# omarkhursheed/whisper-sae

Hardware: AMD Instinct MI355X
Metric: activations/sec through SAE train step (d=384->3072, k=32) (higher is better)
Workload: dtype bf16; 1 GPU; BASELINE.json configs[1]: TopKSAE 384->3072 k=32 train step, synthetic activations resident in the HBM ring buffer; batch_per_gpu=16384, global_batch=16384, ring_rows_per_gpu=4194304, parallelism=dp1

## Files before the change

whisper-sae_amd/csrc/wsae_common.h:

```cpp
#pragma once

#include <hip/hip_runtime.h>
#include <stdint.h>
#include <stdio.h>

#include "wsae.h"

void wsae_set_error(const char* fmt, ...);

#define WSAE_HIP_CHECK(expr)                                                              \
    do {                                                                                  \
        hipError_t e_ = (expr);                                                           \
        if (e_ != hipSuccess) {                                                           \
            wsae_set_error("%s failed: %s (%s:%d)", #expr, hipGetErrorString(e_), __FILE__, \
                           __LINE__);                                                     \
            return WSAE_ERR_HIP;                                                          \
        }                                                                                 \
    } while (0)

#define WSAE_REQUIRE(cond, ...)          \
    do {                                 \
        if (!(cond)) {                   \
            wsae_set_error(__VA_ARGS__); \
            return WSAE_ERR_INVALID;     \
        }                                \
    } while (0)

#define WSAE_LAUNCH_CHECK()                                                                  \
    do {                                                                                     \
        hipError_t e_ = hipGetLastError();                                                   \
        if (e_ != hipSuccess) {                                                              \
            wsae_set_error("kernel launch failed: %s (%s:%d)", hipGetErrorString(e_), __FILE__, \
                           __LINE__);                                                        \
            return WSAE_ERR_HIP;                                                             \
        }                                                                                    \
    } while (0)

typedef __bf16 bf16_t;
typedef __bf16 bf16x8 __attribute__((ext_vector_type(8)));
typedef __bf16 bf16x4 __attribute__((ext_vector_type(4)));
typedef float f32x16 __attribute__((ext_vector_type(16)));
typedef float f32x4 __attribute__((ext_vector_type(4)));
typedef float f32x2 __attribute__((ext_vector_type(2)));
typedef __bf16 bf16x2 __attribute__((ext_vector_type(2)));

static inline int64_t ceil_div64(int64_t a, int64_t b) { return (a + b - 1) / b; }
static inline int ceil_div(int a, int b) { return (a + b - 1) / b; }
static inline int64_t align256(int64_t b) { return (b + 255) & ~(int64_t)255; }
__host__ __device__ __forceinline__ int64_t min64(int64_t a, int64_t b) { return a < b ? a : b; }

#define WSAE_MAX_PARTIALS 1024
#define WSAE_WGRAD_MAX_SPLIT 8

struct wsae_prof {
    unsigned mask;
    int max_samples;
    int count[WSAE_K_COUNT];
    hipEvent_t* ev[WSAE_K_COUNT];
};

struct wsae_ctx {
    wsae_prof prof;
    int D, H, K, maxB, prec, device;
    const float* relu_l1w;
    int loss_cols;
    int cus;
    int comm_reserve;
    int64_t P;
    int64_t off[5];
    bf16_t* We_bf16;
    bf16_t* WdT_bf16;
    float* c_fold;
    void* xb;
    void* xT;
    void* gT;
    float* g;
    bf16_t* gb;
    int g_is_bf16;
    int xT_valid;
    int g32_valid;
    float* pre;
    float* smax;
    int smax_valid;
    uint32_t* tmin;
    int tmin_cur;
    int strip_predict;
    int wgrad_sparse;
    float tg_fixed_s;
    int pred_valid;
    const void* pred_x;
    const int32_t* pred_rows;
    float* part_loss;
    float* part_l0;
    float* part_dbd;
    float* part_sq;
    float* colnorm;
    float* wg_slabs;
    float* dbe_slab;
    float* dbpre_part;
    uint32_t* ent_pos;
    void* ent_hid;
    void* ent_dpre;
    int32_t* ent_off;
    int ent_valid;
    const float* ent_vals;
    int ent_B;
    const float* wire_dec_vals;
    int wire_dec_B;
    int32_t* counters;
    int32_t* dead_list;
    int32_t* row_order;
    int resample_max_rows;
    int relu_fp8;
    void* relu_ws;
    int relu_x_B;
    int relu_g_B;
    float* fired;
    const float* wire_metrics;
    int n_dec_blocks;
    int n_sq_parts;
    float* dbd2;
    int32_t* btk_ws;
    int btk_k;
    int btk_mode;
    wsae_batch_topk_state* btk_state;
    size_t ws_bytes;
};

#define WSAE_PROF_BEGIN(ctx, id, st)                                                          \
    const bool prof_on_##id = ((ctx)->prof.mask >> (id)) & 1u &&                               \
                              (ctx)->prof.count[id] < (ctx)->prof.max_samples;                 \
    if (prof_on_##id) (void)hipEventRecord((ctx)->prof.ev[id][2 * (ctx)->prof.count[id]], st)
#define WSAE_PROF_END(ctx, id, st)                                                            \
    if (prof_on_##id) {                                                                       \
        (void)hipEventRecord((ctx)->prof.ev[id][2 * (ctx)->prof.count[id] + 1], st);           \
        (ctx)->prof.count[id]++;                                                              \
    }

#ifdef __HIPCC__

#define WSAE_WAVE 64

template <int M>
__device__ __forceinline__ uint32_t lane_xor_u32(uint32_t x, int lane) {
    if constexpr (M == 1) return (uint32_t)__builtin_amdgcn_update_dpp(0, (int)x, 0xB1, 0xF, 0xF, false);
    else if constexpr (M == 2) return (uint32_t)__builtin_amdgcn_update_dpp(0, (int)x, 0x4E, 0xF, 0xF, false);
    else if constexpr (M == 4) {
        const uint32_t up = (uint32_t)__builtin_amdgcn_update_dpp(0, (int)x, 0x104, 0xF, 0xF, false);
        const uint32_t dn = (uint32_t)__builtin_amdgcn_update_dpp(0, (int)x, 0x114, 0xF, 0xF, false);
        return (lane & 4) ? dn : up;
    } else if constexpr (M == 8) return (uint32_t)__builtin_amdgcn_update_dpp(0, (int)x, 0x128, 0xF, 0xF, false);
    else if constexpr (M == 16) {
        const auto r = __builtin_amdgcn_permlane16_swap((int)x, (int)x, false, false);
        return (uint32_t)((lane & 16) ? r[0] : r[1]);
    } else {
        static_assert(M == 32, "lane_xor_u32: M must be a power of two <= 32");
        const auto r = __builtin_amdgcn_permlane32_swap((int)x, (int)x, false, false);
        return (uint32_t)((lane & 32) ? r[0] : r[1]);
    }
}

__device__ __forceinline__ float wave_sum(float v) {
    const int lane = threadIdx.x & 63;
    v += __uint_as_float(lane_xor_u32<32>(__float_as_uint(v), lane));
    v += __uint_as_float(lane_xor_u32<16>(__float_as_uint(v), lane));
    v += __uint_as_float(lane_xor_u32<8>(__float_as_uint(v), lane));
    v += __uint_as_float(lane_xor_u32<4>(__float_as_uint(v), lane));
    v += __uint_as_float(lane_xor_u32<2>(__float_as_uint(v), lane));
    v += __uint_as_float(lane_xor_u32<1>(__float_as_uint(v), lane));
    return v;
}
__device__ __forceinline__ float wave_max(float v) {
    const int lane = threadIdx.x & 63;
    v = fmaxf(v, __uint_as_float(lane_xor_u32<32>(__float_as_uint(v), lane)));
    v = fmaxf(v, __uint_as_float(lane_xor_u32<16>(__float_as_uint(v), lane)));
    v = fmaxf(v, __uint_as_float(lane_xor_u32<8>(__float_as_uint(v), lane)));
    v = fmaxf(v, __uint_as_float(lane_xor_u32<4>(__float_as_uint(v), lane)));
    v = fmaxf(v, __uint_as_float(lane_xor_u32<2>(__float_as_uint(v), lane)));
    v = fmaxf(v, __uint_as_float(lane_xor_u32<1>(__float_as_uint(v), lane)));
    return v;
}
__device__ __forceinline__ int wave_sum_i(int v) {
    const int lane = threadIdx.x & 63;
    v += (int)lane_xor_u32<32>((uint32_t)v, lane);
    v += (int)lane_xor_u32<16>((uint32_t)v, lane);
    v += (int)lane_xor_u32<8>((uint32_t)v, lane);
    v += (int)lane_xor_u32<4>((uint32_t)v, lane);
    v += (int)lane_xor_u32<2>((uint32_t)v, lane);
    v += (int)lane_xor_u32<1>((uint32_t)v, lane);
    return v;
}
__device__ __forceinline__ int wave_min_i(int v) {
    const int lane = threadIdx.x & 63;
    int o;
    o = (int)lane_xor_u32<32>((uint32_t)v, lane); v = o < v ? o : v;
    o = (int)lane_xor_u32<16>((uint32_t)v, lane); v = o < v ? o : v;
    o = (int)lane_xor_u32<8>((uint32_t)v, lane); v = o < v ? o : v;
    o = (int)lane_xor_u32<4>((uint32_t)v, lane); v = o < v ? o : v;
    o = (int)lane_xor_u32<2>((uint32_t)v, lane); v = o < v ? o : v;
    o = (int)lane_xor_u32<1>((uint32_t)v, lane); v = o < v ? o : v;
    return v;
}

__device__ __forceinline__ float lane_f32(float x, int lane) {
    return __int_as_float(__builtin_amdgcn_readlane(__float_as_int(x), lane));
}
__device__ __forceinline__ double lane_f64(double x, int lane) {
    const long long b = __double_as_longlong(x);
    const unsigned lo = (unsigned)__builtin_amdgcn_readlane((int)(unsigned)b, lane);
    const unsigned hi = (unsigned)__builtin_amdgcn_readlane((int)(unsigned)(b >> 32), lane);
    return __longlong_as_double((long long)(((unsigned long long)hi << 32) | lo));
}

__device__ __forceinline__ float block_sum(float v, float* scratch) {
    v = wave_sum(v);
    const int lane = threadIdx.x & 63, w = threadIdx.x >> 6, nw = blockDim.x >> 6;
    __syncthreads();
    if (lane == 0) scratch[w] = v;
    __syncthreads();
    float r = 0.f;
    if (threadIdx.x == 0)
        for (int i = 0; i < nw; ++i) r += scratch[i];
    return r;
}

#define TICKET_GROUPS 32
#define TICKET_WORDS (1 + TICKET_GROUPS)
__device__ __forceinline__ bool grid_ticket(unsigned long long* t, unsigned payload, unsigned* total) {
    const unsigned nblk = gridDim.x * gridDim.y;
    const unsigned bid = blockIdx.y * gridDim.x + blockIdx.x;
    const unsigned ngrp = nblk < TICKET_GROUPS ? nblk : TICKET_GROUPS;
    const unsigned grp = bid % ngrp;
    const unsigned gsz = (nblk - grp + ngrp - 1) / ngrp;
    const unsigned long long add = (1ull << 32) | payload;
    const unsigned long long o1 = __hip_atomic_fetch_add(t + 1 + grp, add, __ATOMIC_RELAXED, __HIP_MEMORY_SCOPE_AGENT);
    if ((unsigned)(o1 >> 32) != gsz - 1) return false;
    __hip_atomic_store(t + 1 + grp, 0ull, __ATOMIC_RELAXED, __HIP_MEMORY_SCOPE_AGENT);
    const unsigned long long add2 = (1ull << 32) | (unsigned)((o1 + add) & 0xFFFFFFFFull);
    const unsigned long long o2 = __hip_atomic_fetch_add(t, add2, __ATOMIC_RELAXED, __HIP_MEMORY_SCOPE_AGENT);
    if ((unsigned)(o2 >> 32) != ngrp - 1) return false;
// ... 83 lines not shown
```

whisper-sae_amd/csrc/wsae_ctx.hip:

```cpp
#include <stdarg.h>
#include <stdlib.h>
#include <string.h>

#include <new>

#include "wsae_common.h"
#include "wsae_topk.h"
#include <cstdlib>
#include <vector>

static thread_local char g_err[512] = "";
static void prof_free(wsae_ctx* c);

void wsae_set_error(const char* fmt, ...) {
    va_list ap;
    va_start(ap, fmt);
    vsnprintf(g_err, sizeof(g_err), fmt, ap);
    va_end(ap);
}

extern "C" const char* wsae_last_error(void) { return g_err; }
extern "C" int wsae_version(void) { return WSAE_VERSION; }

extern "C" int64_t wsae_param_count(int32_t D, int32_t H) {
    return 2 * (int64_t)D * H + H + 2 * (int64_t)D;
}

extern "C" int wsae_param_offsets(int32_t D, int32_t H, int64_t off[5]) {
    WSAE_REQUIRE(off != nullptr && D > 0 && H > 0, "wsae_param_offsets: bad arguments");
    off[0] = 0;
    off[1] = (int64_t)D * H;
    off[2] = 2 * (int64_t)D * H;
    off[3] = off[2] + H;
    off[4] = off[3] + D;
    return WSAE_OK;
}

namespace {
struct DeviceGuard {
    int prev = -1;
    bool good = false;
    explicit DeviceGuard(int device) {
        if (hipGetDevice(&prev) != hipSuccess) prev = -1;
        good = hipSetDevice(device) == hipSuccess;
    }
    ~DeviceGuard() {
        if (prev >= 0) (void)hipSetDevice(prev);
    }
    bool ok() const { return good; }
};

struct Carver {
    size_t total = 0;
    size_t take(size_t bytes) {
        size_t at = total;
        total += (bytes + 255) & ~(size_t)255;
        return at;
    }
};
}

extern "C" int wsae_ctx_create(const wsae_config* cfg, wsae_ctx** out) {
    WSAE_REQUIRE(cfg && out, "wsae_ctx_create: null argument");
    const int D = cfg->input_dim, H = cfg->hidden_dim, K = cfg->k, maxB = cfg->max_batch;
    WSAE_REQUIRE(D >= 32 && D % 32 == 0 && D <= 2048, "input_dim must be a multiple of 32 in [32,2048], got %d", D);
    WSAE_REQUIRE(H >= 32 && H % 32 == 0, "hidden_dim must be a positive multiple of 32, got %d", H);
    WSAE_REQUIRE(K >= 1 && K <= 128 && K <= H, "k must be in [1, min(128, hidden_dim)], got %d", K);
    WSAE_REQUIRE(maxB >= 1, "max_batch must be >= 1, got %d", maxB);
    WSAE_REQUIRE(cfg->precision == WSAE_PREC_BF16 || cfg->precision == WSAE_PREC_FP32, "unknown precision %d",
                 cfg->precision);
    DeviceGuard guard(cfg->device);
    if (!guard.ok()) {
        wsae_set_error("hipSetDevice(%d) failed", cfg->device);
        return WSAE_ERR_HIP;
    }

    wsae_ctx* c = new (std::nothrow) wsae_ctx();
    if (!c) {
        wsae_set_error("out of host memory");
        return WSAE_ERR_NOMEM;
    }
    memset(c, 0, sizeof(*c));
    c->loss_cols = D;
    c->D = D; c->H = H; c->K = K; c->maxB = maxB; c->prec = cfg->precision; c->device = cfg->device;
    if (hipDeviceGetAttribute(&c->cus, hipDeviceAttributeMultiprocessorCount, cfg->device) != hipSuccess || c->cus < 1)
        c->cus = 256;
    c->P = wsae_param_count(D, H);
    wsae_param_offsets(D, H, c->off);
    c->resample_max_rows = wsae_internal_resample_max_rows(cfg->device);

    const size_t esz = (c->prec == WSAE_PREC_BF16) ? 2 : 4;
    const size_t maxBp = ((size_t)maxB + 127) / 128 * 128;
    Carver cv;
    const size_t o_we = cv.take((size_t)H * D * 2);
    const size_t o_wd = cv.take((size_t)H * D * 2);
    const size_t o_cf = cv.take((size_t)H * 4);
    const size_t o_xb = cv.take((size_t)maxB * D * esz);
    const size_t o_xT = cv.take(maxBp * D * esz);
    const size_t o_gT = cv.take(maxBp * D * esz);
    const size_t o_g = cv.take((size_t)maxB * D * 4);
    const size_t o_gb = cv.take((size_t)maxB * D * 2);
    const size_t o_pre = cv.take((size_t)maxB * H * 4);
    const size_t o_sm = cv.take((size_t)maxB * ((H + 15) / 16) * 4);
    const size_t o_pl = cv.take(WSAE_MAX_PARTIALS * 4);
    const size_t o_p0 = cv.take(WSAE_MAX_PARTIALS * 4);
    const size_t o_pd = cv.take((size_t)WSAE_MAX_PARTIALS * D * 4);
    const size_t o_ps = cv.take((WSAE_MAX_PARTIALS + 64) * 4);
    const size_t o_d2 = cv.take((size_t)64 * D * 4);
    const size_t o_cn = cv.take((size_t)H * 4);
    const size_t o_ct = cv.take((16 + 3 * 2 * TICKET_WORDS) * 4);
    const size_t o_ws = cv.take((size_t)WSAE_WGRAD_MAX_SPLIT * 2 * H * D * 4);
    const size_t o_ds = cv.take((size_t)2 * WSAE_WGRAD_MAX_SPLIT * H * 4);
    const size_t o_dp = cv.take((size_t)((H + 31) / 32) * D * 4);
    const size_t o_ep = cv.take((size_t)maxB * K * 4);
    const size_t o_eh = cv.take((size_t)maxB * K * 4);
    const size_t o_ed = cv.take((size_t)maxB * K * 4);
    const size_t o_eo = cv.take((size_t)((maxB + 31) / 32) * ((H + 127) / 128 + 1) * 4);
    const size_t o_dl = cv.take((size_t)H * 4);
    const size_t o_ro = cv.take((size_t)maxB * 4);
    const size_t o_tm = cv.take(TG_WORDS * 4);
    const size_t o_bt = cv.take(wsae_internal_batch_topk_ws_bytes());
    char* base = nullptr;
    hipError_t e = hipMalloc((void**)&base, cv.total);
    if (e != hipSuccess) {
        wsae_set_error("hipMalloc(%zu bytes of workspace) failed: %s", cv.total, hipGetErrorString(e));
        delete c;
        return WSAE_ERR_NOMEM;
    }
    e = hipMemset(base, 0, cv.total);
    if (e != hipSuccess) {
        wsae_set_error("hipMemset failed: %s", hipGetErrorString(e));
        (void)hipFree(base);
        delete c;
        return WSAE_ERR_HIP;
    }
    c->We_bf16 = (bf16_t*)(base + o_we);
    c->WdT_bf16 = (bf16_t*)(base + o_wd);
    c->c_fold = (float*)(base + o_cf);
    c->xb = base + o_xb;
    c->xT = base + o_xT;
    c->gT = base + o_gT;
    c->g = (float*)(base + o_g);
    c->gb = (bf16_t*)(base + o_gb);
    c->pre = (float*)(base + o_pre);
    c->smax = (float*)(base + o_sm);
    c->part_loss = (float*)(base + o_pl);
    c->part_l0 = (float*)(base + o_p0);
    c->part_dbd = (float*)(base + o_pd);
    c->part_sq = (float*)(base + o_ps);
    c->dbd2 = (float*)(base + o_d2);
    c->colnorm = (float*)(base + o_cn);
    c->counters = (int32_t*)(base + o_ct);
    c->wg_slabs = (float*)(base + o_ws);
    c->dbe_slab = (float*)(base + o_ds);
    c->dbpre_part = (float*)(base + o_dp);
    c->ent_pos = (uint32_t*)(base + o_ep);
    c->ent_hid = base + o_eh;
    c->ent_dpre = base + o_ed;
    c->ent_off = (int32_t*)(base + o_eo);
    c->dead_list = (int32_t*)(base + o_dl);
    c->row_order = (int32_t*)(base + o_ro);
    c->tmin = (uint32_t*)(base + o_tm);
    c->btk_ws = (int32_t*)(base + o_bt);
    const char* sp = getenv("WSAE_STRIP_PREDICT");
    c->strip_predict = (sp && sp[0] == '0') ? 0 : 1;
    const char* ws = getenv("WSAE_WGRAD_SPARSE");
    c->wgrad_sparse = (ws && ws[0] == '0') ? 0 : 1;
    const char* ss = getenv("WSAE_STRIP_SAFETY");
    c->tg_fixed_s = ss ? (float)atof(ss) : 0.f;
    c->ws_bytes = cv.total;
    *out = c;
    return WSAE_OK;
}

extern "C" int wsae_ctx_destroy(wsae_ctx* ctx) {
    if (!ctx) return WSAE_OK;
    prof_free(ctx);
    if (ctx->relu_ws) (void)hipFree(ctx->relu_ws);
    if (ctx->We_bf16) (void)hipFree((void*)ctx->We_bf16);
    delete ctx;
    return WSAE_OK;
}

static const char* const k_names[WSAE_K_COUNT] = {"stage_batch", "encode_gemm", "topk", "decode", "bucket", "wgrad",
                                                  "wgrad_reduce", "sqnorm", "adamw", "rownorm", "prepare", "dead_scan"};

extern "C" const char* wsae_kernel_name(int32_t id) { return (id >= 0 && id < WSAE_K_COUNT) ? k_names[id] : "?"; }

static void prof_free(wsae_ctx* c) {
    for (int k = 0; k < WSAE_K_COUNT; ++k) {
        if (c->prof.ev[k]) {
            for (int i = 0; i < 2 * c->prof.max_samples; ++i) (void)hipEventDestroy(c->prof.ev[k][i]);
            delete[] c->prof.ev[k];
            c->prof.ev[k] = nullptr;
        }
        c->prof.count[k] = 0;
    }
    c->prof.mask = 0;
    c->prof.max_samples = 0;
}

extern "C" int wsae_profile_disable(wsae_ctx* ctx) {
    WSAE_REQUIRE(ctx, "wsae_profile_disable: null ctx");
    prof_free(ctx);
    return WSAE_OK;
}

extern "C" int wsae_profile_enable(wsae_ctx* ctx, int32_t kernel_id, int32_t max_samples) {
    WSAE_REQUIRE(ctx && kernel_id >= -1 && kernel_id < WSAE_K_COUNT && max_samples >= 1 && max_samples <= 65536,
                 "wsae_profile_enable: bad argument");
    prof_free(ctx);
    ctx->prof.max_samples = max_samples;
    for (int k = 0; k < WSAE_K_COUNT; ++k) {
        if (kernel_id != -1 && kernel_id != k) continue;
        ctx->prof.ev[k] = new (std::nothrow) hipEvent_t[2 * (size_t)max_samples];
        if (!ctx->prof.ev[k]) {
            wsae_set_error("out of host memory");
            return WSAE_ERR_NOMEM;
        }
        for (int i = 0; i < 2 * max_samples; ++i) WSAE_HIP_CHECK(hipEventCreate(&ctx->prof.ev[k][i]));
        ctx->prof.mask |= 1u << k;
    }
    return WSAE_OK;
}

extern "C" int wsae_profile_read(wsae_ctx* ctx, int32_t kernel_id, int32_t* n_launches, double* total_ms) {
    WSAE_REQUIRE(ctx && kernel_id >= 0 && kernel_id < WSAE_K_COUNT && n_launches && total_ms,
                 "wsae_profile_read: bad argument");
    *n_launches = 0;
    *total_ms = 0.0;
    if (!ctx->prof.ev[kernel_id]) return WSAE_OK;
    const int n = ctx->prof.count[kernel_id];
    double tot = 0.0;
    for (int i = 0; i < n; ++i) {
        WSAE_HIP_CHECK(hipEventSynchronize(ctx->prof.ev[kernel_id][2 * i + 1]));
        float ms = 0.f;
        WSAE_HIP_CHECK(hipEventElapsedTime(&ms, ctx->prof.ev[kernel_id][2 * i], ctx->prof.ev[kernel_id][2 * i + 1]));
        tot += ms;
    }
    *n_launches = n;
    *total_ms = tot;
    return WSAE_OK;
}

extern "C" int wsae_ctx_set_fired(wsae_ctx* ctx, float* fired) {
    WSAE_REQUIRE(ctx, "wsae_ctx_set_fired: null ctx");
    ctx->fired = fired;
    return WSAE_OK;
}

static uint32_t host_f32_ord(float f) {
    uint32_t u;
    memcpy(&u, &f, 4);
    return (u & 0x80000000u) ? ~u : (u | 0x80000000u);
}
extern "C" int wsae_ctx_set_strip_predict(wsae_ctx* ctx, int32_t on, float assume_store_threshold) {
    WSAE_REQUIRE(ctx, "wsae_ctx_set_strip_predict: null ctx");
    ctx->strip_predict = on ? 1 : 0;
    ctx->pred_valid = 0;
    WSAE_HIP_CHECK(hipDeviceSynchronize());
    const bool forget = assume_store_threshold != assume_store_threshold;
    const float one = 1.0f;
    uint32_t hdr[3] = {forget ? 0u : host_f32_ord(assume_store_threshold), 0u, 0u};
    if (!forget) memcpy(&hdr[1], &one, 4);
    uint32_t* prev = ctx->tmin + ctx->tmin_cur * TG_GROUP_WORDS;
    WSAE_HIP_CHECK(hipMemset(prev, 0, TG_GROUP_WORDS * 4));
    WSAE_HIP_CHECK(hipMemset(ctx->tmin + ((ctx->tmin_cur + 2) % 3) * TG_GROUP_WORDS, 0, TG_GROUP_WORDS * 4));
    WSAE_HIP_CHECK(hipMemcpy(prev, hdr, sizeof(hdr), hipMemcpyHostToDevice));
    return WSAE_OK;
}
extern "C" int wsae_ctx_strip_stats(wsae_ctx* ctx, int64_t* refilled_rows, float* last_min_threshold, float* margin) {
    WSAE_REQUIRE(ctx && refilled_rows && last_min_threshold && margin, "wsae_ctx_strip_stats: null argument");
    std::vector<uint32_t> h(TG_WORDS);
    WSAE_HIP_CHECK(hipDeviceSynchronize());
    WSAE_HIP_CHECK(hipMemcpy(h.data(), ctx->tmin, h.size() * 4, hipMemcpyDeviceToHost));
    *refilled_rows = (int64_t)h[TG_REFILLED];
    uint32_t o = 0xFFFFFFFFu;
    for (int i = 0; i < TG_SLOTS; ++i) {
        const uint32_t s = h[ctx->tmin_cur * TG_GROUP_WORDS + i * TG_SLOT_STRIDE];
        if (s != 0u && s < o) o = s;
    }
    float f = NAN;
    if (o != 0u && o != 0xFFFFFFFFu) {
        const uint32_t u = (o & 0x80000000u) ? (o & 0x7FFFFFFFu) : ~o;
        memcpy(&f, &u, 4);
    }
    *last_min_threshold = f;
    memcpy(margin, &h[ctx->tmin_cur * TG_GROUP_WORDS + TG_HDR_S], 4);
    return WSAE_OK;
}

extern "C" int wsae_ctx_set_wire_metrics(wsae_ctx* ctx, const float* loss_l0) {
    WSAE_REQUIRE(ctx, "wsae_ctx_set_wire_metrics: null ctx");
    ctx->wire_metrics = loss_l0;
    return WSAE_OK;
}

extern "C" int wsae_ctx_set_loss_cols(wsae_ctx* ctx, int32_t cols) {
    WSAE_REQUIRE(ctx && cols >= 1 && cols <= ctx->D, "wsae_ctx_set_loss_cols: columns must be in [1, input_dim]");
    ctx->loss_cols = cols;
    return WSAE_OK;
}

extern "C" size_t wsae_ctx_workspace_bytes(const wsae_ctx* ctx) { return ctx ? ctx->ws_bytes : 0; }

__global__ void __launch_bounds__(256) prepare_kernel(const float* __restrict__ We, const float* __restrict__ WdT,
                                                      const float* __restrict__ be, const float* __restrict__ bpre,
                                                      bf16_t* __restrict__ We16, bf16_t* __restrict__ WdT16,
                                                      float* __restrict__ cfold, int H, int D) {
    const int lane = threadIdx.x & 63;
    const int h = blockIdx.x * 4 + (threadIdx.x >> 6);
    if (h >= H) return;
    const float* row = We + (int64_t)h * D;
    bf16_t* orow = We16 + (int64_t)h * D;
    const float* drow = WdT + (int64_t)h * D;
    bf16_t* odrow = WdT16 + (int64_t)h * D;
    float dot = 0.f;
    for (int d = lane * 4; d < D; d += 256) {
        const float4 wd = *(const float4*)(drow + d);
        bf16x4 o, e;
// ... 31 lines not shown
```

whisper-sae_amd/csrc/wsae_decode_mfma.hip:

```cpp
#include "wsae_chunk_sort.h"
#include "wsae_common.h"
#include "wsae_decode_epilogue.h"
#include "wsae_mfma.h"

#ifdef WSAE_DM_STAMPS
__device__ unsigned long long dm_stamp_sum[8];
#define DM_T(i)                                                                                     \
    {                                                                                               \
        __builtin_amdgcn_sched_barrier(0);                                                          \
        unsigned long long t_;                                                                      \
        asm volatile("s_memtime %0\n\ts_waitcnt lgkmcnt(0)" : "=s"(t_)::"memory");                  \
        __builtin_amdgcn_sched_barrier(0);                                                          \
        dm_acc[i] += t_ - dm_last;                                                                  \
        dm_last = t_;                                                                               \
    }
extern "C" int wsae_debug_stamps(double* out, int reset) {
    unsigned long long h[8];
    if (hipMemcpyFromSymbol(h, HIP_SYMBOL(dm_stamp_sum), sizeof(h)) != hipSuccess) return -1;
    for (int i = 0; i < 8; ++i) out[i] = (double)h[i];
    if (reset) {
        unsigned long long z[8] = {0, 0, 0, 0, 0, 0, 0, 0};
        (void)hipMemcpyToSymbol(HIP_SYMBOL(dm_stamp_sum), z, sizeof(z));
    }
    return 0;
}
#else
#define DM_T(i) __builtin_amdgcn_sched_barrier(0);
#endif

typedef __attribute__((address_space(3))) bf16x4 lds_bf16x4;

__device__ __forceinline__ int dm_sw(int j) { return (j & 15) ^ ((j & 1) ? 12 : 0); }

__device__ __forceinline__ bf16x8 tr_frag(const char* a0, const char* a1) {
    const bf16x4 lo = __builtin_amdgcn_ds_read_tr16_b64_v4bf16((lds_bf16x4*)a0);
    const bf16x4 hi = __builtin_amdgcn_ds_read_tr16_b64_v4bf16((lds_bf16x4*)a1);
    return __builtin_shufflevector(lo, hi, 0, 1, 2, 3, 4, 5, 6, 7);
}

template <int N>
__device__ __forceinline__ void dma_piece(const void* base, const uint32_t (&off)[N], uint32_t lds) {
    static_assert(N == 8 || N == 16, "a piece is 32 or 64 rows");
    const uint32_t l0 = __builtin_amdgcn_readfirstlane(lds);
    uint32_t keep;
#define DP1(i) "global_load_lds_dwordx4 %" #i ", %[b]\n\ts_add_u32 m0, m0, 0x400\n\ts_nop 0\n\t"
    if constexpr (N == 8) {
        asm volatile("s_mov_b32 %[k], m0\n\ts_mov_b32 m0, %[l]\n\ts_nop 0\n\t" DP1(2) DP1(3) DP1(4) DP1(5) DP1(6) DP1(7) DP1(8) DP1(9)
                     "s_mov_b32 m0, %[k]"
                     : [k] "=&s"(keep)
                     : [l] "s"(l0), "v"(off[0]), "v"(off[1]), "v"(off[2]), "v"(off[3]), "v"(off[4]), "v"(off[5]), "v"(off[6]),
                       "v"(off[7]), [b] "s"(base)
                     : "memory");
    } else {
        asm volatile("s_mov_b32 %[k], m0\n\ts_mov_b32 m0, %[l]\n\ts_nop 0\n\t" DP1(2) DP1(3) DP1(4) DP1(5) DP1(6) DP1(7) DP1(8) DP1(9)
                     DP1(10) DP1(11) DP1(12) DP1(13) DP1(14) DP1(15) DP1(16) DP1(17) "s_mov_b32 m0, %[k]"
                     : [k] "=&s"(keep)
                     : [l] "s"(l0), "v"(off[0]), "v"(off[1]), "v"(off[2]), "v"(off[3]), "v"(off[4]), "v"(off[5]), "v"(off[6]),
                       "v"(off[7]), "v"(off[8]), "v"(off[9]), "v"(off[10]), "v"(off[11]), "v"(off[12]), "v"(off[13]),
                       "v"(off[14]), "v"(off[15]), [b] "s"(base)
                     : "memory");
    }
#undef DP1
}

template <int N>
__device__ __forceinline__ void vm_wait() {
    if constexpr (N == 0) asm volatile("s_waitcnt vmcnt(0)" ::: "memory");
    else if constexpr (N == 8) asm volatile("s_waitcnt vmcnt(8)" ::: "memory");
    else {
        static_assert(N == 16, "vm_wait: one piece of 32 or 64 rows in flight");
        asm volatile("s_waitcnt vmcnt(16)" ::: "memory");
    }
}

__host__ __device__ constexpr int dm_wave_bytes(int KS, int D) {
    return 2 * (32 * KS) * 256 + 2 * 2 * (32 * KS) * 4 + D * 2 + 128 * 4;
}

template <int KS, int NSUB, int XDT, bool BWD, int NW>
__global__ void __launch_bounds__(64 * NW, (KS == 1 && NSUB <= 3) ? 2 : 1)
decode_mfma_kernel(const bf16_t* __restrict__ WdT, const float* __restrict__ bd, const float* __restrict__ bpre,
                   const void* __restrict__ x, const int32_t* __restrict__ rows, const float* __restrict__ vals,
                   const int32_t* __restrict__ idx, int B, int K, float* __restrict__ recon_out, float* __restrict__ dpre,
                   float* __restrict__ g32_out, bf16_t* __restrict__ gb_out, int64_t* __restrict__ last_activated,
                   float* __restrict__ fired, const int64_t* __restrict__ step_count, float* __restrict__ part_loss,
                   float* __restrict__ part_l0, float* __restrict__ part_dbd, int32_t* __restrict__ ticket,
                   wsae_stats* __restrict__ stats, int loss_cols, int ntiles, int tw, uint32_t* __restrict__ ent_pos,
                   bf16_t* __restrict__ ent_hid, bf16_t* __restrict__ ent_dpre, int32_t* __restrict__ ent_off) {
    static_assert(NW == 4 || (NW == 8 && BWD), "the chunked form exists for the training backward only");
    constexpr int D = 128 * NSUB;
    constexpr int KP = 32 * KS;
    constexpr int E = KP / 4;
    constexpr int SLOT = KP * 256;
    constexpr int WAVE_BYTES = dm_wave_bytes(KS, D);
    static_assert(WAVE_BYTES % 16 == 0, "per-wave LDS regions stay 16-byte aligned");
    extern __shared__ __attribute__((aligned(16))) char smem[];
    const int lane = threadIdx.x & 63, wave = threadIdx.x >> 6;
    const int n = lane & 15, grp = lane >> 4;
    const uint32_t piece_mask[3] = {n == 0 ? 0xFFFFFFFFu : 0u, n == 1 ? 0xFFFFFFFFu : 0u, n == 2 ? 0xFFFFFFFFu : 0u};
    char* wbase = smem + wave * WAVE_BYTES;
    char* slot0 = wbase;
    char* code = wbase + 2 * SLOT;
    bf16_t* grow = (bf16_t*)(code + 2 * 2 * KP * 4);
    float* stage = (float*)(grow + D);
    float* red = (float*)(smem + NW * WAVE_BYTES);
    int* flag_s = (int*)(red + 8);
    float* dbd_s = (float*)smem;
    const uint32_t slot_lds = (uint32_t)(uintptr_t)(__attribute__((address_space(3))) char*)slot0;

    for (int i = lane; i < 2 * 2 * KP; i += 64) ((int*)code)[i] = 0;
    f32x2 bsum2[NSUB];
#pragma unroll
    for (int s = 0; s < NSUB; ++s) {
        const float2 a = *(const float2*)(bd + 128 * s + 2 * lane), p = *(const float2*)(bpre + 128 * s + 2 * lane);
        bsum2[s] = f32x2{a.x + p.x, a.y + p.y};
    }

    const float scale = 2.0f / ((float)B * (float)loss_cols);
    const int64_t step = (last_activated && step_count) ? *step_count : 0;
    constexpr bool x_bf16 = XDT == WSAE_DT_BF16;
    int tr_off[KS][2], tr_swz[2], a2_off[2 * KS], a2_swz[2 * KS];
    {
        const int i = n >> 2, p = n & 3;
#pragma unroll
        for (int h2 = 0; h2 < 2; ++h2) {
            const int jr = 8 * grp + i + 4 * h2;
            tr_swz[h2] = (dm_sw(jr) ^ (p >> 1)) << 4;
#pragma unroll
            for (int q = 0; q < KS; ++q) tr_off[q][h2] = (32 * q + jr) * 256 + 8 * (p & 1);
        }
#pragma unroll
        for (int m = 0; m < 2 * KS; ++m) {
            a2_off[m] = (16 * m + n) * 256;
            a2_swz[m] = (dm_sw(16 * m + n) ^ grp) << 4;
        }
    }
    float loss_acc = 0.f;
    int l0_acc = 0;
    f32x2 dbd[NSUB];
#pragma unroll
    for (int s = 0; s < NSUB; ++s) dbd[s] = f32x2{0.f, 0.f};

    auto get_code = [&](int bb, int cb) {
        float* vs = (float*)(code + cb * 2 * KP * 4);
        int32_t* is = (int32_t*)(vs + KP);
        if (lane < K) {
            vs[lane] = vals[(int64_t)bb * K + lane];
            is[lane] = idx[(int64_t)bb * K + lane];
        }
    };
    auto sources = [&](int cb, uint32_t (&rp)[E]) {
        const int32_t* is = (const int32_t*)(code + cb * 2 * KP * 4) + KP;
#pragma unroll
        for (int e = 0; e < E; ++e) {
            const int j = 4 * e + grp;
            rp[e] = (uint32_t)is[j] * (uint32_t)D + 8u * (uint32_t)(n ^ dm_sw(j));
        }
    };
    auto issue = [&](const uint32_t (&rp)[E], int s, int slot) {
        asm volatile("s_waitcnt lgkmcnt(0)" ::: "memory");
        uint32_t off[E];
#pragma unroll
        for (int e = 0; e < E; ++e) off[e] = 2u * rp[e] + 256u * (uint32_t)s;
        dma_piece<E>(WdT, off, slot_lds + slot * SLOT);
    };

    const int b_first = NW == 8 ? blockIdx.x * 64 + wave : blockIdx.x * 4 + wave;
    const int b_step = NW == 8 ? 8 : gridDim.x * 4;
    const int b_end = NW == 8 ? min(B, (int)blockIdx.x * 64 + 64) : B;
    int buf = 0, par = 0;
    int64_t src_next = 0;
    uint32_t rowp[E];
#ifdef WSAE_DM_STAMPS
    unsigned long long dm_acc[8] = {0, 0, 0, 0, 0, 0, 0, 0}, dm_last = __builtin_amdgcn_s_memtime();
#endif
    if (b_first < b_end) {
        src_next = rows ? (int64_t)rows[b_first] : (int64_t)b_first;
        get_code(b_first, 0);
        sources(0, rowp);
        issue(rowp, 0, 0);
        if (NSUB > 1) issue(rowp, 1, 1);
    }
    DM_T(0)
    for (int b = b_first; b < b_end; b += b_step) {
        const float* vs = (const float*)(code + buf * 2 * KP * 4);
        const int32_t* is = (const int32_t*)(vs + KP);
        const bool more = b + b_step < b_end;
        {
            const float v = lane < KP ? vs[lane < KP ? lane : 0] : 0.f;
            const bool on = lane < K && v > 0.f;
            l0_acc += __popcll(__ballot(on));
            if (on && last_activated) {
                const int f = is[lane];
                last_activated[f] = step;
                if (fired) fired[f] = 1.f;
            }
        }
        const int64_t src = src_next;
        if (more) src_next = rows ? (int64_t)rows[b + b_step] : (int64_t)(b + b_step);
        uint32_t xraw[NSUB][x_bf16 ? 1 : 2];
#pragma unroll
        for (int s = 0; s < NSUB; ++s) {
            if constexpr (x_bf16) {
                xraw[s][0] = *(const uint32_t*)((const uint16_t*)x + src * D + 128 * s + 2 * lane);
            } else {
                const uint2 t2 = *(const uint2*)((const uint32_t*)x + src * D + 128 * s + 2 * lane);
                xraw[s][0] = t2.x;
                xraw[s][1] = t2.y;
            }
        }
        bf16x8 a1[KS];
#pragma unroll
        for (int q = 0; q < KS; ++q) {
            const float4 v0 = *(const float4*)(vs + 32 * q + 8 * grp), v1 = *(const float4*)(vs + 32 * q + 8 * grp + 4);
            const float vv[8] = {v0.x, v0.y, v0.z, v0.w, v1.x, v1.y, v1.z, v1.w};
            uint32_t w4[4];
#pragma unroll
            for (int p2 = 0; p2 < 4; ++p2) {
                const float a = __builtin_amdgcn_fmed3f(vv[2 * p2], 0.f, INFINITY);
                const float b = __builtin_amdgcn_fmed3f(vv[2 * p2 + 1], 0.f, INFINITY);
                bf16x2 h2;
                h2[0] = (bf16_t)a; h2[1] = (bf16_t)b;
                const uint32_t hb = __builtin_bit_cast(uint32_t, h2);
                const float ra = a - __uint_as_float(hb << 16), rb = b - __uint_as_float(hb & 0xFFFF0000u);
                bf16x2 l2;
                l2[0] = (bf16_t)ra; l2[1] = (bf16_t)rb;
                const uint32_t lb = __builtin_bit_cast(uint32_t, l2);
                const float sa = ra - __uint_as_float(lb << 16), sb = rb - __uint_as_float(lb & 0xFFFF0000u);
                bf16x2 t2;
                t2[0] = (bf16_t)sa; t2[1] = (bf16_t)sb;
                const uint32_t tb = __builtin_bit_cast(uint32_t, t2);
                w4[p2] = (hb & piece_mask[0]) | (lb & piece_mask[1]) | (tb & piece_mask[2]);
            }
            typedef uint32_t u32x4 __attribute__((ext_vector_type(4)));
            const u32x4 wv = {w4[0], w4[1], w4[2], w4[3]};
            a1[q] = __builtin_bit_cast(bf16x8, wv);
        }
        DM_T(1)
        uint32_t rowp_n[E];
        if (more) {
            get_code(b + b_step, buf ^ 1);
            sources(buf ^ 1, rowp_n);
        } else {
#pragma unroll
            for (int e = 0; e < E; ++e) rowp_n[e] = rowp[e];
        }
        if (NSUB == 1 && more) issue(rowp_n, 0, par ^ 1);
        DM_T(2)
        if (NSUB == 1 && more) vm_wait<E>(); else vm_wait<0>();
        DM_T(3)

        f32x4 acc2[2 * KS];
#pragma unroll
        for (int m = 0; m < 2 * KS; ++m) acc2[m] = f32x4{0.f, 0.f, 0.f, 0.f};
#pragma unroll
        for (int s = 0; s < NSUB; ++s) {
            if (s >= 2 || (s == 1 && NSUB == 2)) {
                if (s + 1 < NSUB || more) vm_wait<E>(); else vm_wait<0>();
            }
            DM_T(4)
            const int sl = (par + s) & 1;
            const char* slot = slot0 + sl * SLOT;
#pragma unroll
            for (int th = 0; th < 2; ++th) {
                f32x4 acc[4];
#pragma unroll
                for (int u = 0; u < 4; ++u) {
                    const int t = 4 * th + u;
                    acc[u] = f32x4{0.f, 0.f, 0.f, 0.f};
#pragma unroll
                    for (int q = 0; q < KS; ++q) {
                        const bf16x8 bf = tr_frag(slot + tr_off[q][0] + ((32 * t) ^ tr_swz[0]), slot + tr_off[q][1] + ((32 * t) ^ tr_swz[1]));
                        acc[u] = __builtin_amdgcn_mfma_f32_16x16x32_bf16(a1[q], bf, acc[u], 0, 0, 0);
                    }
                }
                if (lane < 16) {
#pragma unroll
                    for (int u = 0; u < 4; ++u) stage[16 * (4 * th + u) + n] = (acc[u][0] + acc[u][1]) + acc[u][2];
                }
            }
            {
                const float2 sm = *(const float2*)(stage + 2 * lane);
                const float rec0 = sm.x + bsum2[s][0], rec1 = sm.y + bsum2[s][1];
                float x0, x1;
                if constexpr (x_bf16) {
                    x0 = __uint_as_float(xraw[s][0] << 16);
                    x1 = __uint_as_float(xraw[s][0] & 0xFFFF0000u);
                } else {
                    x0 = __uint_as_float(xraw[s][0]);
                    x1 = __uint_as_float(xraw[s][1]);
                }
                const float r0 = rec0 - x0, r1 = rec1 - x1;
                const float g0 = r0 * scale, g1 = r1 * scale;
                loss_acc = fmaf(r0, r0, fmaf(r1, r1, loss_acc));
                dbd[s][0] += g0;
                dbd[s][1] += g1;
                bf16x2 gb2;
                gb2[0] = (bf16_t)g0;
                gb2[1] = (bf16_t)g1;
                const int col = 128 * s + 2 * lane;
                *(bf16x2*)(grow + col) = gb2;
                if (recon_out) *(float2*)(recon_out + (int64_t)b * D + col) = make_float2(rec0, rec1);
                if (BWD) {
                    *(bf16x2*)(gb_out + (int64_t)b * D + col) = gb2;
                    if (g32_out) *(float2*)(g32_out + (int64_t)b * D + col) = make_float2(g0, g1);
                }
            }
            DM_T(5)
            if (BWD) {
#pragma unroll
                for (int kk = 0; kk < 4; ++kk) {
                    const bf16x8 gf = *(const bf16x8*)(grow + 128 * s + 32 * kk + 8 * grp);
#pragma unroll
                    for (int m = 0; m < 2 * KS; ++m) {
                        const bf16x8 af = *(const bf16x8*)(slot + a2_off[m] + ((64 * kk) ^ a2_swz[m]));
                        acc2[m] = __builtin_amdgcn_mfma_f32_16x16x32_bf16(af, gf, acc2[m], 0, 0, 0);
                    }
                }
            }
            if (NSUB >= 2) {
                if (s + 2 < NSUB) issue(rowp, s + 2, sl);
                else if (more) issue(rowp_n, s + 2 - NSUB, sl);
            }
            DM_T(6)
        }
        if (BWD) {
#pragma unroll
            for (int m = 0; m < 2 * KS; ++m) {
                const int j = 16 * m + 4 * grp + (n & 3);
                const float d0 = (n & 2) ? ((n & 1) ? acc2[m][3] : acc2[m][2]) : ((n & 1) ? acc2[m][1] : acc2[m][0]);
                float out = vs[j] > 0.f ? d0 : 0.f;
                out = (float)(bf16_t)out;
                if (n < 4 && j < K) dpre[(int64_t)b * K + j] = out;
            }
        }
        par = (par + NSUB) & 1;
        buf ^= 1;
#pragma unroll
        for (int e = 0; e < E; ++e) rowp[e] = rowp_n[e];
        DM_T(7)
    }
#ifdef WSAE_DM_STAMPS
    if (lane == 0)
        for (int i = 0; i < 8; ++i) atomicAdd(&dm_stamp_sum[i], dm_acc[i]);
#endif

    vm_wait<0>();
    __syncthreads();
    if constexpr (NW == 8) {
        int* cnt = (int*)smem;
        int* cur = cnt + 512;
        constexpr int EB = 8;
        const int tid = threadIdx.x;
        const int c0 = (int)blockIdx.x * 64;
        const int nent = (b_end - c0) * K;
        const int64_t base = (int64_t)c0 * K;
        int f[EB], tl[EB];
        float v[EB], dp[EB];
#pragma unroll
        for (int j = 0; j < EB; ++j) {
            const int e = min(tid + 512 * j, nent - 1);
            f[j] = idx[base + e];
            v[j] = vals[base + e];
            dp[j] = dpre[base + e];
        }
        for (int t = tid; t < ntiles; t += 512) cnt[t] = 0;
        __syncthreads();
#pragma unroll
        for (int j = 0; j < EB; ++j) {
            tl[j] = f[j] / tw;
            if (tid + 512 * j < nent) atomicAdd(&cnt[tl[j]], 1);
        }
        __syncthreads();
        if (tid < 64) {
            int carry = 0;
            for (int t0 = 0; t0 < ntiles; t0 += 64) {
                const int t = t0 + tid;
                const int c = t < ntiles ? cnt[t] : 0;
                int incl = c;
#pragma unroll
                for (int o = 1; o < 64; o <<= 1) {
                    const int nn = __shfl_up(incl, o, 64);
                    if (tid >= o) incl += nn;
                }
                if (t < ntiles) {
                    cur[t] = carry + incl - c;
                    ent_off[(int64_t)blockIdx.x * (ntiles + 1) + t] = (int)base + carry + incl - c;
                }
                carry += __shfl(incl, 63, 64);
            }
            if (tid == 0) ent_off[(int64_t)blockIdx.x * (ntiles + 1) + ntiles] = (int)base + carry;
        }
        __syncthreads();
#pragma unroll
        for (int j = 0; j < EB; ++j) {
            const int e = tid + 512 * j;
            if (e >= nent) continue;
            const int p = atomicAdd(&cur[tl[j]], 1);
            ent_pos[base + p] = ent_pack(f[j] - tl[j] * tw, e / K);
            ent_hid[base + p] = (bf16_t)(v[j] > 0.f ? v[j] : 0.f);
            ent_dpre[base + p] = (bf16_t)dp[j];
        }
        __syncthreads();
    }
    if (BWD) {
#pragma unroll
        for (int s = 0; s < NSUB; ++s) *(float2*)(dbd_s + wave * D + 128 * s + 2 * lane) = make_float2(dbd[s][0], dbd[s][1]);
    }
    __syncthreads();
    decode_block_epilogue<BWD, NW>(loss_acc, l0_acc, dbd_s, D, B, loss_cols, red, flag_s, part_loss, part_l0, part_dbd, ticket, stats);
}

template <typename F>
static int resident_per_cu(F kernel, size_t sh) {
    int n = 0;
    if (hipOccupancyMaxActiveBlocksPerMultiprocessor(&n, kernel, 256, sh) != hipSuccess || n < 1) n = 1;
    return n;
}

void wsae_internal_wgrad_tiling(const wsae_ctx* c, int* tile_width, int* ntiles);

template <int KS, int NSUB, int XDT>
static int dm_launch(wsae_ctx* c, const float* params, const void* x, const int32_t* rows, const float* vals,
                     const int32_t* idx, int B, float* recon, int want_bwd, float* dpre, float* g32, int64_t* last_activated,
                     const int64_t* step_count, wsae_stats* stats, hipStream_t st) {
    const size_t sh = 4 * (size_t)dm_wave_bytes(KS, 128 * NSUB) + 12 * 4;
    static const int per_cu[2] = {resident_per_cu(decode_mfma_kernel<KS, NSUB, XDT, false, 4>, sh),
                                  resident_per_cu(decode_mfma_kernel<KS, NSUB, XDT, true, 4>, sh)};
    int tw = 0, ntiles = 0;
    wsae_internal_wgrad_tiling(c, &tw, &ntiles);
#define DM_ARGS c->WdT_bf16, params + c->off[3], params + c->off[4], x, rows, vals, idx, B, c->K, recon, dpre, g32, \
                c->gb, last_activated, c->fired, step_count, c->part_loss, c->part_l0, c->part_dbd,                       \
                c->counters + 16 + 2 * TICKET_WORDS, stats, c->loss_cols, ntiles, tw, c->ent_pos, (bf16_t*)c->ent_hid,   \
                (bf16_t*)c->ent_dpre, c->ent_off
    const int nchunks = ceil_div(B, 64);
    c->ent_valid = 0;
    if constexpr (KS == 1 && NSUB <= 3) {
        if (want_bwd && dpre && NSUB == 3 && nchunks >= c->cus && nchunks <= WSAE_MAX_PARTIALS && ntiles <= 512 &&
            c->K * 64 <= 4096) {
            const size_t sh8 = 8 * (size_t)dm_wave_bytes(KS, 128 * NSUB) + 12 * 4;
            decode_mfma_kernel<KS, NSUB, XDT, true, 8><<<nchunks, 512, sh8, st>>>(DM_ARGS);
            c->ent_valid = 1;
            c->ent_vals = vals;
            c->ent_B = B;
            return nchunks;
        }
    }
    const int nblk = min(ceil_div(B, 4), min(per_cu[want_bwd ? 1 : 0] * c->cus, WSAE_MAX_PARTIALS));
    if (want_bwd) decode_mfma_kernel<KS, NSUB, XDT, true, 4><<<nblk, 256, sh, st>>>(DM_ARGS);
    else decode_mfma_kernel<KS, NSUB, XDT, false, 4><<<nblk, 256, sh, st>>>(DM_ARGS);
#undef DM_ARGS
    return nblk;
}

bool wsae_internal_decode_mfma_ok(const wsae_ctx* c) {
    if (c->prec != WSAE_PREC_BF16 || c->D % 128 || c->K > 64) return false;
    const int ns = c->D / 128;
    if (c->K > 32) return ns == 3 || ns == 6 || ns == 10;
    return ns == 1 || ns == 2 || ns == 3 || ns == 6 || ns == 10;
}

int wsae_internal_decode_mfma(wsae_ctx* c, const float* params, const void* x, int x_dtype, const int32_t* rows,
                              const float* vals, const int32_t* idx, int B, float* recon, int want_bwd, float* dpre,
                              int want_g32, int64_t* last_activated, const int64_t* step_count, wsae_stats* stats,
                              hipStream_t st) {
    const int ns = c->D / 128, ks = c->K <= 32 ? 1 : 2;
    int nblk = 0;
    float* g32 = want_g32 ? c->g : nullptr;
#define DM_CASE(KS_, NS_)                                                                                              \
    nblk = x_dtype == WSAE_DT_BF16                                                                                     \
               ? dm_launch<KS_, NS_, WSAE_DT_BF16>(c, params, x, rows, vals, idx, B, recon, want_bwd, dpre, g32,        \
                                                   last_activated, step_count, stats, st)                               \
               : dm_launch<KS_, NS_, WSAE_DT_F32>(c, params, x, rows, vals, idx, B, recon, want_bwd, dpre, g32,         \
                                                  last_activated, step_count, stats, st);                               \
    break
    WSAE_PROF_BEGIN(c, WSAE_K_DECODE, st);
    if (ks == 1) {
        switch (ns) {
            case 1: DM_CASE(1, 1);
            case 2: DM_CASE(1, 2);
            case 3: DM_CASE(1, 3);
            case 6: DM_CASE(1, 6);
            default: DM_CASE(1, 10);
        }
    } else {
        switch (ns) {
            case 3: DM_CASE(2, 3);
            case 6: DM_CASE(2, 6);
            default: DM_CASE(2, 10);
        }
    }
    WSAE_PROF_END(c, WSAE_K_DECODE, st);
#undef DM_CASE
    WSAE_LAUNCH_CHECK();
    c->n_dec_blocks = nblk;
    c->g_is_bf16 = 1;
    c->g32_valid = want_g32 ? 1 : 0;
    return WSAE_OK;
}
```

Before: 75.02 million activations/s.

## Prefetch decode row headers and x rows into LDS one row ahead

Adds a prefetch variant of the MFMA decode kernel for the k<=32, D=384, bf16 shape. It streams each row's top-k values and indices plus the input x row into LDS with direct global-to-LDS loads a row ahead, and reads row indices through scalar loads. The goal is to hide global load latency for codes and x behind the MFMA work and to restructure the vmcnt waits. It is on by default behind an env flag, uses extra LDS per wave, and depends on finely ordered waitcnt accounting.

```diff
diff --git a/whisper-sae_amd/csrc/wsae_common.h b/whisper-sae_amd/csrc/wsae_common.h
--- a/whisper-sae_amd/csrc/wsae_common.h
+++ b/whisper-sae_amd/csrc/wsae_common.h
@@ -86,6 +86,7 @@
     int tmin_cur;
     int strip_predict;
     int wgrad_sparse;
+    int decode_prefetch;
     float tg_fixed_s;
     int pred_valid;
     const void* pred_x;
diff --git a/whisper-sae_amd/csrc/wsae_ctx.hip b/whisper-sae_amd/csrc/wsae_ctx.hip
--- a/whisper-sae_amd/csrc/wsae_ctx.hip
+++ b/whisper-sae_amd/csrc/wsae_ctx.hip
@@ -166,6 +166,8 @@
     c->strip_predict = (sp && sp[0] == '0') ? 0 : 1;
     const char* ws = getenv("WSAE_WGRAD_SPARSE");
     c->wgrad_sparse = (ws && ws[0] == '0') ? 0 : 1;
+    const char* dp = getenv("WSAE_DECODE_PREFETCH");
+    c->decode_prefetch = (dp && dp[0] == '0') ? 0 : 1;
     const char* ss = getenv("WSAE_STRIP_SAFETY");
     c->tg_fixed_s = ss ? (float)atof(ss) : 0.f;
     c->ws_bytes = cv.total;
diff --git a/whisper-sae_amd/csrc/wsae_decode_mfma.hip b/whisper-sae_amd/csrc/wsae_decode_mfma.hip
--- a/whisper-sae_amd/csrc/wsae_decode_mfma.hip
+++ b/whisper-sae_amd/csrc/wsae_decode_mfma.hip
@@ -4,7 +4,8 @@
 #include "wsae_mfma.h"
 
 #ifdef WSAE_DM_STAMPS
-__device__ unsigned long long dm_stamp_sum[8];
+#define DM_NSTAMP 12
+__device__ unsigned long long dm_stamp_sum[DM_NSTAMP];
 #define DM_T(i)                                                                                     \
     {                                                                                               \
         __builtin_amdgcn_sched_barrier(0);                                                          \
@@ -14,12 +15,13 @@
         dm_acc[i] += t_ - dm_last;                                                                  \
         dm_last = t_;                                                                               \
     }
+extern "C" int wsae_debug_stamps_count() { return DM_NSTAMP; }
 extern "C" int wsae_debug_stamps(double* out, int reset) {
-    unsigned long long h[8];
+    unsigned long long h[DM_NSTAMP];
     if (hipMemcpyFromSymbol(h, HIP_SYMBOL(dm_stamp_sum), sizeof(h)) != hipSuccess) return -1;
-    for (int i = 0; i < 8; ++i) out[i] = (double)h[i];
+    for (int i = 0; i < DM_NSTAMP; ++i) out[i] = (double)h[i];
     if (reset) {
-        unsigned long long z[8] = {0, 0, 0, 0, 0, 0, 0, 0};
+        unsigned long long z[DM_NSTAMP] = {};
         (void)hipMemcpyToSymbol(HIP_SYMBOL(dm_stamp_sum), z, sizeof(z));
     }
     return 0;
@@ -65,19 +67,21 @@
 
 template <int N>
 __device__ __forceinline__ void vm_wait() {
-    if constexpr (N == 0) asm volatile("s_waitcnt vmcnt(0)" ::: "memory");
-    else if constexpr (N == 8) asm volatile("s_waitcnt vmcnt(8)" ::: "memory");
-    else {
-        static_assert(N == 16, "vm_wait: one piece of 32 or 64 rows in flight");
-        asm volatile("s_waitcnt vmcnt(16)" ::: "memory");
-    }
+    static_assert(N >= 0 && N < 64, "vmcnt is a 6-bit count");
+    asm volatile("s_waitcnt vmcnt(%0)" ::"n"(N) : "memory");
 }
 
 __host__ __device__ constexpr int dm_wave_bytes(int KS, int D) {
     return 2 * (32 * KS) * 256 + 2 * 2 * (32 * KS) * 4 + D * 2 + 128 * 4;
 }
-
-template <int KS, int NSUB, int XDT, bool BWD, int NW>
+__host__ __device__ constexpr bool dm_prefetch_shape(int KS, int NSUB, int XDT) {
+    return KS == 1 && NSUB == 3 && XDT == WSAE_DT_BF16;
+}
+__host__ __device__ constexpr int dm_wave_bytes_x(int KS, int NSUB, int XDT) {
+    return dm_wave_bytes(KS, 128 * NSUB) + (dm_prefetch_shape(KS, NSUB, XDT) ? 128 * NSUB * 2 : 0);
+}
+
+template <int KS, int NSUB, int XDT, bool BWD, int NW, bool PF = false>
 __global__ void __launch_bounds__(64 * NW, (KS == 1 && NSUB <= 3) ? 2 : 1)
 decode_mfma_kernel(const bf16_t* __restrict__ WdT, const float* __restrict__ bd, const float* __restrict__ bpre,
                    const void* __restrict__ x, const int32_t* __restrict__ rows, const float* __restrict__ vals,
@@ -88,11 +92,12 @@
                    wsae_stats* __restrict__ stats, int loss_cols, int ntiles, int tw, uint32_t* __restrict__ ent_pos,
                    bf16_t* __restrict__ ent_hid, bf16_t* __restrict__ ent_dpre, int32_t* __restrict__ ent_off) {
     static_assert(NW == 4 || (NW == 8 && BWD), "the chunked form exists for the training backward only");
+    static_assert(!PF || dm_prefetch_shape(KS, NSUB, XDT), "the header stream is written for k <= 32, D = 384, bf16 x");
     constexpr int D = 128 * NSUB;
     constexpr int KP = 32 * KS;
     constexpr int E = KP / 4;
     constexpr int SLOT = KP * 256;
-    constexpr int WAVE_BYTES = dm_wave_bytes(KS, D);
+    constexpr int WAVE_BYTES = dm_wave_bytes_x(KS, NSUB, XDT);
     static_assert(WAVE_BYTES % 16 == 0, "per-wave LDS regions stay 16-byte aligned");
     extern __shared__ __attribute__((aligned(16))) char smem[];
     const int lane = threadIdx.x & 63, wave = threadIdx.x >> 6;
@@ -103,6 +108,7 @@
     char* code = wbase + 2 * SLOT;
     bf16_t* grow = (bf16_t*)(code + 2 * 2 * KP * 4);
     float* stage = (float*)(grow + D);
+    const uint32_t* xrow = (const uint32_t*)(stage + 128);
     float* red = (float*)(smem + NW * WAVE_BYTES);
     int* flag_s = (int*)(red + 8);
     float* dbd_s = (float*)smem;
@@ -114,6 +120,9 @@
     for (int s = 0; s < NSUB; ++s) {
         const float2 a = *(const float2*)(bd + 128 * s + 2 * lane), p = *(const float2*)(bpre + 128 * s + 2 * lane);
         bsum2[s] = f32x2{a.x + p.x, a.y + p.y};
+        if constexpr (PF) {
+            asm volatile("" : "+v"(bsum2[s][0]), "+v"(bsum2[s][1]));
+        }
     }
 
     const float scale = 2.0f / ((float)B * (float)loss_cols);
@@ -164,17 +173,43 @@
         for (int e = 0; e < E; ++e) off[e] = 2u * rp[e] + 256u * (uint32_t)s;
         dma_piece<E>(WdT, off, slot_lds + slot * SLOT);
     };
-
-    const int b_first = NW == 8 ? blockIdx.x * 64 + wave : blockIdx.x * 4 + wave;
+    auto hdr_code = [&](int bb, int cb) {
+        if (lane < 16 && (lane & 7) < (K >> 2)) {
+            const char* src = (lane < 8 ? (const char*)vals : (const char*)idx) + ((int64_t)bb * K + 4 * (lane & 7)) * 4;
+            glds16(src, slot_lds + 2 * SLOT + cb * 2 * KP * 4);
+        }
+    };
+    auto hdr_x = [&](int src) {
+        if (lane < D / 8) glds16((const char*)x + (int64_t)src * (2 * D) + 16 * lane, slot_lds + WAVE_BYTES - 2 * D);
+    };
+    auto row_of = [&](int bb) -> int {
+        typedef const __attribute__((address_space(4))) int32_t* crows_t;
+        const int ub = __builtin_amdgcn_readfirstlane(bb);
+        return rows ? ((crows_t)(uintptr_t)rows)[ub] : ub;
+    };
+
+    const int b_first0 = NW == 8 ? blockIdx.x * 64 + wave : blockIdx.x * 4 + wave;
+    const int b_first = PF ? __builtin_amdgcn_readfirstlane(b_first0) : b_first0;
     const int b_step = NW == 8 ? 8 : gridDim.x * 4;
     const int b_end = NW == 8 ? min(B, (int)blockIdx.x * 64 + 64) : B;
     int buf = 0, par = 0;
     int64_t src_next = 0;
     uint32_t rowp[E];
 #ifdef WSAE_DM_STAMPS
-    unsigned long long dm_acc[8] = {0, 0, 0, 0, 0, 0, 0, 0}, dm_last = __builtin_amdgcn_s_memtime();
+    unsigned long long dm_acc[DM_NSTAMP] = {}, dm_last = __builtin_amdgcn_s_memtime();
 #endif
-    if (b_first < b_end) {
+    int src_n1 = 0, src_n2 = 0;
+    if constexpr (PF) {
+        if (b_first < b_end) {
+            src_n1 = b_first + b_step < b_end ? row_of(b_first + b_step) : 0;
+            asm volatile("s_waitcnt lgkmcnt(0)" ::: "memory");
+            hdr_code(b_first, 0);
+            hdr_x(row_of(b_first));
+            vm_wait<1>();
+            sources(0, rowp);
+            issue(rowp, 0, 0);
+        }
+    } else if (b_first < b_end) {
         src_next = rows ? (int64_t)rows[b_first] : (int64_t)b_first;
         get_code(b_first, 0);
         sources(0, rowp);
@@ -186,6 +221,7 @@
         const float* vs = (const float*)(code + buf * 2 * KP * 4);
         const int32_t* is = (const int32_t*)(vs + KP);
         const bool more = b + b_step < b_end;
+        if constexpr (PF) src_n2 = b + 2 * b_step < b_end ? row_of(b + 2 * b_step) : 0;
         {
             const float v = lane < KP ? vs[lane < KP ? lane : 0] : 0.f;
             const bool on = lane < K && v > 0.f;
@@ -196,12 +232,14 @@
                 if (fired) fired[f] = 1.f;
             }
         }
+        if constexpr (PF) issue(rowp, 1, par ^ 1);
         const int64_t src = src_next;
-        if (more) src_next = rows ? (int64_t)rows[b + b_step] : (int64_t)(b + b_step);
+        if (!PF && more) src_next = rows ? (int64_t)rows[b + b_step] : (int64_t)(b + b_step);
         uint32_t xraw[NSUB][x_bf16 ? 1 : 2];
 #pragma unroll
         for (int s = 0; s < NSUB; ++s) {
-            if constexpr (x_bf16) {
+            if constexpr (PF) {
+            } else if constexpr (x_bf16) {
                 xraw[s][0] = *(const uint32_t*)((const uint16_t*)x + src * D + 128 * s + 2 * lane);
             } else {
                 const uint2 t2 = *(const uint2*)((const uint32_t*)x + src * D + 128 * s + 2 * lane);
@@ -238,6 +276,21 @@
         }
         DM_T(1)
         uint32_t rowp_n[E];
+        if constexpr (PF) {
+#pragma unroll
+            for (int e = 0; e < E; ++e) rowp_n[e] = rowp[e];
+            (void)src;
+            vm_wait<E>();
+            DM_T(8)
+#pragma unroll
+            for (int s = 0; s < NSUB; ++s) xraw[s][0] = xrow[64 * s + lane];
+            asm volatile("s_waitcnt lgkmcnt(0)" ::: "memory");
+            if (more) {
+                hdr_code(b + b_step, buf ^ 1);
+                hdr_x(src_n1);
+            }
+            DM_T(2)
+        } else {
         if (more) {
             get_code(b + b_step, buf ^ 1);
             sources(buf ^ 1, rowp_n);
@@ -249,13 +302,17 @@
         DM_T(2)
         if (NSUB == 1 && more) vm_wait<E>(); else vm_wait<0>();
         DM_T(3)
+        }
 
         f32x4 acc2[2 * KS];
 #pragma unroll
         for (int m = 0; m < 2 * KS; ++m) acc2[m] = f32x4{0.f, 0.f, 0.f, 0.f};
 #pragma unroll
         for (int s = 0; s < NSUB; ++s) {
-            if (s >= 2 || (s == 1 && NSUB == 2)) {
+            if (PF && s == 1) {
+                if (more) vm_wait<E + 2>(); else vm_wait<E>();
+                DM_T(9)
+            } else if (s >= 2 || (s == 1 && NSUB == 2)) {
                 if (s + 1 < NSUB || more) vm_wait<E>(); else vm_wait<0>();
             }
             DM_T(4)
@@ -318,9 +375,15 @@
                     }
                 }
             }
+            if (PF && s == NSUB - 2 && more) {
+                DM_T(6)
+                vm_wait<E + 1>();
+                DM_T(10)
+                sources(buf ^ 1, rowp_n);
+            }
             if (NSUB >= 2) {
                 if (s + 2 < NSUB) issue(rowp, s + 2, sl);
-                else if (more) issue(rowp_n, s + 2 - NSUB, sl);
+                else if (more && !(PF && s == NSUB - 1)) issue(rowp_n, s + 2 - NSUB, sl);
             }
             DM_T(6)
         }
@@ -336,13 +399,14 @@
         }
         par = (par + NSUB) & 1;
         buf ^= 1;
+        if constexpr (PF) src_n1 = src_n2;
 #pragma unroll
         for (int e = 0; e < E; ++e) rowp[e] = rowp_n[e];
         DM_T(7)
     }
 #ifdef WSAE_DM_STAMPS
     if (lane == 0)
-        for (int i = 0; i < 8; ++i) atomicAdd(&dm_stamp_sum[i], dm_acc[i]);
+        for (int i = 0; i < DM_NSTAMP; ++i) atomicAdd(&dm_stamp_sum[i], dm_acc[i]);
 #endif
 
     vm_wait<0>();
@@ -424,9 +488,12 @@
 static int dm_launch(wsae_ctx* c, const float* params, const void* x, const int32_t* rows, const float* vals,
                      const int32_t* idx, int B, float* recon, int want_bwd, float* dpre, float* g32, int64_t* last_activated,
                      const int64_t* step_count, wsae_stats* stats, hipStream_t st) {
-    const size_t sh = 4 * (size_t)dm_wave_bytes(KS, 128 * NSUB) + 12 * 4;
+    const size_t sh = 4 * (size_t)dm_wave_bytes_x(KS, NSUB, XDT) + 12 * 4;
     static const int per_cu[2] = {resident_per_cu(decode_mfma_kernel<KS, NSUB, XDT, false, 4>, sh),
                                   resident_per_cu(decode_mfma_kernel<KS, NSUB, XDT, true, 4>, sh)};
+    constexpr bool PFS = dm_prefetch_shape(KS, NSUB, XDT);
+    const bool pf = PFS && want_bwd && c->decode_prefetch && c->K % 4 == 0 &&
+                    (((uintptr_t)vals | (uintptr_t)idx | (uintptr_t)x) & 15) == 0;
     int tw = 0, ntiles = 0;
     wsae_internal_wgrad_tiling(c, &tw, &ntiles);
 #define DM_ARGS c->WdT_bf16, params + c->off[3], params + c->off[4], x, rows, vals, idx, B, c->K, recon, dpre, g32, \
@@ -438,8 +505,9 @@
     if constexpr (KS == 1 && NSUB <= 3) {
         if (want_bwd && dpre && NSUB == 3 && nchunks >= c->cus && nchunks <= WSAE_MAX_PARTIALS && ntiles <= 512 &&
             c->K * 64 <= 4096) {
-            const size_t sh8 = 8 * (size_t)dm_wave_bytes(KS, 128 * NSUB) + 12 * 4;
-            decode_mfma_kernel<KS, NSUB, XDT, true, 8><<<nchunks, 512, sh8, st>>>(DM_ARGS);
+            const size_t sh8 = 8 * (size_t)dm_wave_bytes_x(KS, NSUB, XDT) + 12 * 4;
+            if (pf) decode_mfma_kernel<KS, NSUB, XDT, true, 8, PFS><<<nchunks, 512, sh8, st>>>(DM_ARGS);
+            else decode_mfma_kernel<KS, NSUB, XDT, true, 8><<<nchunks, 512, sh8, st>>>(DM_ARGS);
             c->ent_valid = 1;
             c->ent_vals = vals;
             c->ent_B = B;
@@ -447,7 +515,8 @@
         }
     }
     const int nblk = min(ceil_div(B, 4), min(per_cu[want_bwd ? 1 : 0] * c->cus, WSAE_MAX_PARTIALS));
-    if (want_bwd) decode_mfma_kernel<KS, NSUB, XDT, true, 4><<<nblk, 256, sh, st>>>(DM_ARGS);
+    if (pf) decode_mfma_kernel<KS, NSUB, XDT, true, 4, PFS><<<nblk, 256, sh, st>>>(DM_ARGS);
+    else if (want_bwd) decode_mfma_kernel<KS, NSUB, XDT, true, 4><<<nblk, 256, sh, st>>>(DM_ARGS);
     else decode_mfma_kernel<KS, NSUB, XDT, false, 4><<<nblk, 256, sh, st>>>(DM_ARGS);
 #undef DM_ARGS
     return nblk;
```

Result: no change. 75.65 million activations/s, median of 6 (+0.8%).
